# rpng/online_lang_splatting

Measured on AMD Instinct MI355X. Metric: rasterizer fwd+bwd frames/sec @500k Gaussians, 1200x680, 15-dim lang, higher is better.
Workload: dtype f32

## Files before the change

online_lang_splatting_amd/csrc/k_binning.hip:

```cpp
#include "olsr_device.h"
#include "olsr_kernels.h"
#include "olsr_loss_device.h"

namespace olsr {

constexpr int SCAN_THREADS = 256;
constexpr int SCAN_ITEMS = SCAN_CHUNK / SCAN_THREADS;

struct LoadPlain {
  const u32* p;
  __device__ __forceinline__ u32 operator()(int64_t i) const { return p[i]; }
};
struct LoadGather {
  const u32* vals;
  const u32* order;
  __device__ __forceinline__ u32 operator()(int64_t i) const { return vals[order[i]]; }
};

template <class Load>
__global__ __launch_bounds__(SCAN_THREADS) void scan_reduce_kernel(Load ld, int64_t n, u32* partials) {
  const int64_t base = (int64_t)blockIdx.x * SCAN_CHUNK + (int64_t)threadIdx.x * SCAN_ITEMS;
  u32 s = 0;
#pragma unroll
  for (int k = 0; k < SCAN_ITEMS; ++k)
// ... 324 lines not shown
    off[k] = run;
    run += n[k];
    nbig += (n[k] > EMIT_BIG) ? 1u : 0u;
    nmid += (n[k] > OLSR_MID_FOOTPRINT && n[k] <= EMIT_BIG) ? 1u : 0u;
  }
#pragma unroll
  for (int k = 0; k < EO_PER; ++k) {
    if (n[k] > 0) {
      inst_start[g[k]] = off[k];
      c_off[ci] = off[k];
      c_gid[ci] = g[k];
      for (u32 j = (off[k] + eb_out - 1u) >> eb_shift; (j << eb_shift) < off[k] + n[k]; ++j)
        win_start[j] = ci;
      ++ci;
    }
  }
  if ((r0 <= P - 1 && P - 1 < r0 + EO_PER) || (P == 0 && b == 0 && threadIdx.x == 0)) counters[CNT_EMITTERS] = (int32_t)ci;
  u32 slot = block_list_base<EO_T / 64>(nbig, &counters[CNT_BIG_LIST], s_lsum, &s_lbase);
#pragma unroll
  for (int k = 0; k < EO_PER; ++k)
    if (n[k] > EMIT_BIG) big_list[slot++] = make_uint4(g[k], off[k], n[k], 0u);
  u32 mslot = block_list_base<EO_T / 64>(nmid, &counters[CNT_MID_LIST], s_lsum, &s_lbase);
#pragma unroll
  for (int k = 0; k < EO_PER; ++k)
    if (n[k] > OLSR_MID_FOOTPRINT && n[k] <= EMIT_BIG) big_list[(u32)P_true - 1u - (mslot++)] = make_uint4(g[k], off[k], n[k], 0u);
}

struct EbGauss {
  float4 e0;
  float4 e1;
  uint4 m;
};

template <int TILE>
__global__ __launch_bounds__(EB_T) void emit_balanced_kernel(
    const u32* __restrict__ order, const u32* __restrict__ rank_off, const u32* __restrict__ win_start,
    const float4* __restrict__ emit_rec, int ellipse, int W, int H, int gx, const int32_t* __restrict__ counters,
    u32* __restrict__ keys, u32* __restrict__ inst_gid, u32 eb_out) {
  __shared__ EbGauss s_gs[EB_T];
  __shared__ u32 s_g[EB_T], s_first[EB_T], s_rowoff[EB_T];
  __shared__ uint8_t s_owner[EB_ROWCAP];
  __shared__ u32 s_w[EB_T / 64];
  __shared__ u32 s_flag;
  if (counters[CNT_OVERFLOW] != 0 || counters[CNT_SYNC_ERROR] != 0) return;
  const u32 R = (u32)counters[CNT_INSTANCES_EFF];
  const int P = counters[CNT_EMITTERS];
  const u32 o0 = blockIdx.x * eb_out;
  if (o0 >= R) return;
  const u32 o1 = min(o0 + eb_out, R);
  const int tid = threadIdx.x, lane = tid & 63;

  const int r_lo = (int)win_start[blockIdx.x];
  auto load_rank = [&](int r, u32& off, u32& end, u32& g) {
    off = 0; end = 0; g = 0;
    if (r < P) {
      off = rank_off[r];
      end = (r + 1 < P) ? rank_off[r + 1] : R;
      g = order[r];
    }
  };
  u32 off, end, g;
  load_rank(r_lo + tid, off, end, g);

  for (int rb0 = r_lo;; rb0 += EB_T) {
    const int r = rb0 + tid;
    const bool use = end > off && off < o1 && end > o0;
    u32 nrows = 0;
    if (use) {
      const float4 r0 = emit_rec[2 * (size_t)g], r1 = emit_rec[2 * (size_t)g + 1];
      const u32 yw = __float_as_uint(r1.z), xw = __float_as_uint(r1.w);
      nrows = yw >> 16;
      EbGauss q;
      q.m = make_uint4(0u, xw, yw & 0xFFFFu, off);
      q.e0 = make_float4(0.f, 0.f, 0.f, 0.f);
      q.e1 = make_float4(0.f, 0.f, 0.f, 0.f);
      if (ellipse) {
        const CullEllipse e = cull_setup(r0.x, r0.y, r0.z, r0.w, r1.x, r1.y, 0);
        q.e0 = make_float4(e.px, e.py, e.b, e.inv_a);
        q.e1 = make_float4(e.A, e.det_lo, e.xstar, e.ystar);
        q.m.x = e.exact ? 1u : 0u;
      }
      s_gs[tid] = q;
    }
// ... 25 lines not shown
          owner = (int)s_owner[idx - sbase];
          const EbGauss q = s_gs[owner];
          const int y = (int)q.m.z + (int)(idx - s_rowoff[owner]);
          int xa = (int)(q.m.y & 0xFFFFu), xb = (int)(q.m.y >> 16);
          if (ellipse) {
            CullEllipse e;
            e.px = q.e0.x; e.py = q.e0.y; e.b = q.e0.z; e.inv_a = q.e0.w;
            e.A = q.e1.x; e.det_lo = q.e1.y; e.xstar = q.e1.z; e.ystar = q.e1.w;
            e.ymax = 0.f;
            e.exact = q.m.x != 0u;
            cull_row_span<TILE>(e, xa, xb, y, W, H, xa, xb);
          }
          cnt = (u32)(xb - xa);
          key0 = (u32)(y * gx + xa);
        }
        u32 chunk_total;
        __syncthreads();
        const u32 S = carry + block_excl_scan<EB_T / 64>(cnt, s_w, &chunk_total);
        carry += chunk_total;
        if (live && idx == s_rowoff[owner]) s_first[owner] = S;
        __syncthreads();
        u32 out = 0, gid = 0;
        if (live) {
          out = s_gs[owner].m.w + (S - s_first[owner]);
          gid = s_g[owner];
        }
        const u32 jlo = max(out, o0), jhi = min(out + cnt, o1);
        const bool inside = live && jlo < jhi;
        if (inside && cnt <= EB_SHORT_ROW) {
          for (u32 j = jlo; j < jhi; ++j) {
            keys[j] = key0 + (j - out);
            inst_gid[j] = gid;
          }
        }
        u64 longrows = ballot(inside && cnt > EB_SHORT_ROW);
        while (longrows) {
          const int src = (int)__builtin_ctzll(longrows);
          longrows &= longrows - 1;
          const u32 lo_s = (u32)__shfl((int)jlo, src), hi_s = (u32)__shfl((int)jhi, src);
          const u32 out_s = (u32)__shfl((int)out, src), key_s = (u32)__shfl((int)key0, src);
          const u32 gid_s = (u32)__shfl((int)gid, src);
          for (u32 j = lo_s + (u32)lane; j < hi_s; j += 64) {
            keys[j] = key_s + (j - out_s);
            inst_gid[j] = gid_s;
          }
        }
      }
      __syncthreads();
    }
    if (!more) break;
    off = off_n;
    end = end_n;
    g = g_n;
    __syncthreads();
  }
}

__global__ __launch_bounds__(EMIT_THREADS) void emit_totals_kernel(int P, const u32* __restrict__ order,
                                                                   const u32* __restrict__ inst_count,
                                                                   u64* __restrict__ totals) {
  __shared__ u64 s_w[EMIT_THREADS / 64];
  const int r = (int)(blockIdx.x * EMIT_THREADS + threadIdx.x);
  u64 n = (r < P) ? emit_total_pack(inst_count[order[r]]) : 0ull;
  n = wave_sum(n);
  if ((threadIdx.x & 63) == 0) s_w[threadIdx.x >> 6] = n;
  __syncthreads();
  if (threadIdx.x == 0) {
    u64 t = 0;
    for (int i = 0; i < EMIT_THREADS / 64; ++i) t += s_w[i];
    totals[blockIdx.x] = t;
  }
}
void launch_emit_totals(const uint32_t* order, int P, const uint32_t* inst_count, uint32_t* emit_totals, hipStream_t st) {
  if (P <= 0) return;
  emit_totals_kernel<<<(P + EMIT_THREADS - 1) / EMIT_THREADS, EMIT_THREADS, 0, st>>>(P, order, inst_count,
                                                                                     reinterpret_cast<u64*>(emit_totals));
}

template <int TILE>
static void launch_emit_t(const olsr_scene& s, const FrameDims& d, const GeometryState& g, const BinningState& b,
                          int64_t bin_sync_words, int64_t n_host, const u32* order, const u32* alt_totals,
                          const u32* alt_unless, const int32_t* n_order_dev, hipStream_t st) {
  const int nb = (s.P + EMIT_THREADS - 1) / EMIT_THREADS;
  const int ellipse = (s.binning == OLSR_BINNING_ELLIPSE);
  const u32* totals = g.emit_status;
  uint4* bsync = reinterpret_cast<uint4*>(b.sync_words);
  const int quads = (int)((bin_sync_words + 3) / 4);
  u32* rank_off = g.key_b;
  u32* rank_gid = g.val_b;
  u32* win_start = b.key_b;
  const bool cut_mode = ellipse && s.tile_depth_cut != nullptr;
  const int eb_out = cut_mode ? EB_OUT / 4 : EB_OUT;
  emit_offsets_kernel<<<nb, EO_T, 0, st>>>(s.P, order, g.tiles_touched, g.counters, reinterpret_cast<const u64*>(totals), bsync,
                                           quads, rank_off, rank_gid, win_start, g.inst_start, g.big_list,
                                           (u32)__builtin_ctz((unsigned)eb_out), reinterpret_cast<const u64*>(alt_totals),
                                           alt_unless, n_order_dev);
  const int64_t nblk = (n_host + eb_out - 1) / eb_out;
  if (nblk > 0)
    emit_balanced_kernel<TILE><<<(int)nblk, EB_T, 0, st>>>(rank_gid, rank_off, win_start, g.emit_rec,
                                                           ellipse, d.W, d.H, d.gx, g.counters, b.key_a, b.inst_gid,
                                                           (u32)eb_out);
}

void launch_emit(const olsr_scene& s, const FrameDims& d, const GeometryState& g, const BinningState& b,
                 int64_t bin_sync_words, int64_t n_host, const uint32_t* order, const uint32_t* alt_totals,
                 const uint32_t* alt_unless, const int32_t* n_order_dev, hipStream_t st) {
  if (s.P <= 0) return;
  if (d.tile == 15) launch_emit_t<15>(s, d, g, b, bin_sync_words, n_host, order, alt_totals, alt_unless, n_order_dev, st);
  else launch_emit_t<16>(s, d, g, b, bin_sync_words, n_host, order, alt_totals, alt_unless, n_order_dev, st);
}

__device__ __forceinline__ void load_popc16(const uint8_t* __restrict__ flags, int64_t base, int64_t n, int shift,
                                            u32 mask, u32 (&v)[16]) {
  uint4 q = make_uint4(0u, 0u, 0u, 0u);
  if (base + 16 <= n) {
    q = *reinterpret_cast<const uint4*>(flags + base);
  } else {
    u32 w[4] = {0u, 0u, 0u, 0u};
    for (int k = 0; k < 16; ++k)
      if (base + k < n) w[k >> 2] |= (u32)flags[base + k] << (8 * (k & 3));
    q = make_uint4(w[0], w[1], w[2], w[3]);
  }
  const u32 w4[4] = {q.x, q.y, q.z, q.w};
#pragma unroll
  for (int k = 0; k < 16; ++k) v[k] = (u32)__popc((w4[k >> 2] >> (8 * (k & 3) + shift)) & mask);
}

constexpr int ROWS_THREADS = OLSR_ROWS_THREADS;
static_assert(ROWS_CHUNK == ROWS_THREADS * 16, "one 16-byte load of flags per thread");

struct RowCompactionArgs {
  const uint8_t* flags;
  int64_t n_host;
  const int32_t* n_dev;
  int shift;
  u32 mask;
  u32* rowbase;
  u32* status;
  u32* sync;
  long long row_capacity;
  int32_t* counters;
  int32_t* status_dev;
// ... 332 lines not shown
```

online_lang_splatting_amd/csrc/k_sort.hip:

```cpp
#include <cstdio>
#include <cstdlib>

#include "olsr_device.h"
#include "olsr_kernels.h"

namespace olsr {

constexpr u32 FS_READY = 0x80000000u;
constexpr int FS_T = FUSED_SORT_THREADS;
constexpr int FS_W = FS_T / 64;

typedef unsigned short u16;
constexpr u32 FS_READY16 = 0x8000u;
constexpr u32 FS_READY_PAIR = 0x80008000u;
typedef unsigned int u32x4 __attribute__((ext_vector_type(4)));
__device__ __forceinline__ bool fs_granule_ready(const u32x4& v) {
  return ((v.x & v.y & v.z & v.w) & FS_READY_PAIR) == FS_READY_PAIR;
}

struct FrameHousekeeping {
  const u32* part_rect;
  const u32* part_count;
  int nparts;
  long long capacity;
// ... 229 lines not shown

typedef __attribute__((address_space(3))) u32 lds_u32;
template <int DB>
__device__ __forceinline__ void wave_match_rank(u32 dg, bool valid, u32& rank, u32& pop) {
  const u64 vm = ballot(valid);
  u32 lo = (u32)vm, hi = (u32)(vm >> 32);
#pragma unroll
  for (int bit = 0; bit < DB; ++bit) {
    const u32 b = (dg >> bit) & 1u;
    const u64 bm = ballot(b != 0u);
    const u32 m = 0u - b;
    lo &= ~((u32)bm ^ m);
    hi &= ~((u32)(bm >> 32) ^ m);
  }
  rank = __builtin_amdgcn_mbcnt_hi(hi, __builtin_amdgcn_mbcnt_lo(lo, 0u));
  pop = (u32)__builtin_popcount(lo) + (u32)__builtin_popcount(hi);
}
__device__ __forceinline__ u32 lds_load(const u32* p) {
  return *reinterpret_cast<const volatile lds_u32*>((const lds_u32*)p);
}
__device__ __forceinline__ void lds_store(u32* p, u32 v) { *reinterpret_cast<volatile lds_u32*>((lds_u32*)p) = v; }

constexpr int FSF_IDENTITY = 1, FSF_NO_KEYS = 2, FSF_RANGES = 4, FSF_EMIT_TOTALS = 8;

template <int DB, int KPT, int T>
__global__ __launch_bounds__(T, (T == 1024 ? (KPT <= 2 ? 8 : 4) : (KPT <= 8 ? 8 : 6))) __attribute__((amdgpu_num_sgpr(80))) void sort_pass_kernel(const u32* __restrict__ keys_in,
                                                         const u32* __restrict__ vals_in, int64_t n_host,
                                                         const int32_t* __restrict__ n_dev, int shift,
                                                         const u32* __restrict__ ghist, u16* status, u32* ticket,
                                                         u32* __restrict__ keys_out, u32* __restrict__ vals_out,
                                                         int fsf, uint8_t* __restrict__ flags_clear, u32* ranges,
                                                         const u32* __restrict__ inst_count, u64* emit_totals,
                                                         unsigned long long* timing, int32_t* sync_error, int spin_limit,
                                                         int fault, const u32* __restrict__ run_if) {
  if (run_if != nullptr && __hip_atomic_load(run_if, __ATOMIC_RELAXED, __HIP_MEMORY_SCOPE_AGENT) == 0u) return;
  constexpr int TW = T / 64;
  static_assert(T == 1024 || T == 256, "block sizes of the radix passes");
  constexpr u32 NB = 1u << DB;
  static_assert((int)NB <= T, "a thread per digit");
  constexpr u32 DMASK = NB - 1u;
  constexpr int CHUNK = T * KPT;
  constexpr int C = (int)NB / 8;
  constexpr int RPB = T / C;
  constexpr int U = (DB <= 6) ? 4 : 8;
  extern __shared__ __attribute__((aligned(16))) u32 fs_smem[];
  u32* cnt = fs_smem;
  u32* dstart = cnt + TW * NB;
  u32* gbase = dstart + NB + 4;
  u16* pub = reinterpret_cast<u16*>(gbase + NB);
  u32* ex_key = gbase + NB + NB / 2;
  u32* ex_val = ex_key + CHUNK;
  __shared__ u32 s_bid;
  __shared__ u32 s_w[2 * TW];
  const int tid = threadIdx.x, lane = tid & 63, w = tid >> 6;
  if (tid == 0) s_bid = atomicAdd(ticket, 1u);
  for (u32 i = tid; i < TW * NB; i += T) cnt[i] = 0;
  const u32 gh = ((u32)tid < NB) ? ghist[tid] : 0u;
  const u32 gdig = block_excl_scan<TW>(gh, s_w);
  __syncthreads();
  const u32 b = s_bid;
  FS_STAMP(0);
  if (timing != nullptr && tid == 0) {
    timing[(size_t)b * 8 + 6] = (unsigned long long)(__builtin_amdgcn_s_getreg(63508) & 15);
    timing[(size_t)b * 8 + 7] = (unsigned long long)blockIdx.x;
  }
  const int64_t n = bounded_n(n_host, n_dev);
  const int64_t bbase = (int64_t)b * CHUNK;
  if (__hip_atomic_load(sync_error, __ATOMIC_RELAXED, __HIP_MEMORY_SCOPE_AGENT) != 0) return;
  if (b >= gridDim.x) {
    if (tid == 0) atomicOr(sync_error, 1);
    return;
  }
  if (bbase >= n) return;
  const int64_t wbase = bbase + (int64_t)w * (64 * KPT);

  u32 key[KPT], val[KPT];
#pragma unroll
  for (int r = 0; r < KPT; ++r) {
    const int64_t i = wbase + r * 64 + lane;
    const bool valid = i < n;
    key[r] = valid ? keys_in[i] : 0xFFFFFFFFu;
    val[r] = (fsf & FSF_IDENTITY) ? (u32)i : (valid ? vals_in[i] : 0u);
    if (valid) atomicAdd(&cnt[w * NB + ((key[r] >> shift) & DMASK)], 1u);
    if ((fsf & FSF_IDENTITY) && valid && flags_clear != nullptr) flags_clear[i] = 0;
  }
  __syncthreads();
  FS_STAMP(1);

  const u32 d = (u32)tid;
  u32 c[TW];
// ... 254 lines not shown
}

template <int KPT>
static void launch_sort_small_t(const u32* keys, int n, u32* vals_out, const u32* inst_count, u64* emit_totals,
                                const FrameHousekeeping& h, const u32* run_if, hipStream_t st) {
  constexpr size_t smem = sizeof(u32) * ((size_t)FS_W * 256 + 2 * (size_t)FS_T * KPT);
  static bool attr_set = false;
  if (!attr_set && smem > 64 * 1024) {
    (void)hipFuncSetAttribute(reinterpret_cast<const void*>(&sort_small_kernel<KPT>),
                              hipFuncAttributeMaxDynamicSharedMemorySize, (int)smem);
    attr_set = true;
  }
  sort_small_kernel<KPT><<<1, FS_T, smem, st>>>(keys, n, vals_out, inst_count, emit_totals, h, run_if);
}

struct PassArgs {
  const u32 *kin, *vin;
  int64_t n_host;
  const int32_t* n_dev;
  int shift;
  const u32* ghist;
  u16* status;
  u32* ticket;
  u32 *kout, *vout;
  int fsf;
  uint8_t* flags;
  u32* ranges;
  const u32* inst_count;
  u64* emit_totals;
  int nblk;
  int32_t* sync_error;
  int fault;
  const u32* run_if;
};

template <int DB, int KPT, int T>
static void launch_pass_t(const PassArgs& a, hipStream_t st) {
  constexpr size_t NB = 1u << DB;
  constexpr size_t smem = sizeof(u32) * ((T / 64) * NB + NB + 4 + NB + NB / 2 + 2 * (size_t)T * KPT);
  static bool attr_set = false;
  if (!attr_set && smem > 64 * 1024) {
    (void)hipFuncSetAttribute(reinterpret_cast<const void*>(&sort_pass_kernel<DB, KPT, T>),
                              hipFuncAttributeMaxDynamicSharedMemorySize, (int)smem);
    attr_set = true;
  }
  static bool printed = std::getenv("OLSR_SORT_DEBUG") == nullptr;
  if (!printed) {
    int nb = -1;
    (void)hipOccupancyMaxActiveBlocksPerMultiprocessor(&nb, sort_pass_kernel<DB, KPT, T>, T, smem);
    std::fprintf(stderr, "[olsr] sort_pass_kernel<%d,%d,%d>: %zu B dynamic LDS, occupancy API: %d blocks/CU, grid %d\n", DB,
                 KPT, T, smem, nb, a.nblk);
    printed = true;
  }
  unsigned long long* timing = nullptr;
  if (g_timing.buf && g_timing.launch < g_timing.max_launches && a.nblk <= g_timing.max_blocks)
    timing = g_timing.buf + (size_t)(g_timing.launch++) * g_timing.max_blocks * 8;
  sort_pass_kernel<DB, KPT, T><<<a.nblk, T, smem, st>>>(a.kin, a.vin, a.n_host, a.n_dev, a.shift, a.ghist, a.status,
                                                        a.ticket, a.kout, a.vout, a.fsf, a.flags, a.ranges,
                                                        a.inst_count, a.emit_totals, timing, a.sync_error,
                                                        sort_knobs().spin_limit.load(std::memory_order_relaxed), a.fault,
                                                        a.run_if);
}

template <int DB, int T>
static void launch_pass_kt(int kpt, const PassArgs& a, hipStream_t st) {
  switch (kpt) {
    case 2: launch_pass_t<DB, 2, T>(a, st); break;
    case 4: launch_pass_t<DB, 4, T>(a, st); break;
    case 8: launch_pass_t<DB, 8, T>(a, st); break;
    case 12: launch_pass_t<DB, 12, T>(a, st); break;
    default: launch_pass_t<DB, 16, T>(a, st); break;
  }
}
template <int DB>
static void launch_pass_k(const SortPlan& plan, const PassArgs& a, hipStream_t st) {
  if (plan.threads == 256) launch_pass_kt<DB, 256>(plan.kpt, a, st);
  else launch_pass_kt<DB, 1024>(plan.kpt, a, st);
}

int fused_sort_digit_bits(int bits, int* passes_out) {
  const int passes = (bits + 7) / 8;
  int db = (bits + passes - 1) / passes;
  if (db < 4) db = 4;
  if (passes_out) *passes_out = passes;
  return db;
}

bool fused_sort_applicable(int64_t n_host, int bits) {
  return n_host > 0 && bits <= 32 && fused_sort_fits(n_host);
}

static FrameHousekeeping housekeeping_of(const FusedHouse* house) {
  FrameHousekeeping h{};
  if (house) {
// ... 35 lines not shown
}

void launch_sort_hist(const uint32_t* keys, int64_t n_host, const int32_t* n_dev, int bits, uint32_t* hist,
                      const FusedHouse* house, int threads, hipStream_t st, const uint32_t* run_if,
                      const SortCompaction* compaction) {
  int passes;
  const int db = fused_sort_digit_bits(bits, &passes);
  const FrameHousekeeping h = housekeeping_of(house);
  const int T = threads;
  int64_t nb = (n_host + (int64_t)T * 4 - 1) / ((int64_t)T * 4);
  if (nb < 1) nb = 1;
#ifndef OLSR_HIST_BLOCKS
#define OLSR_HIST_BLOCKS 256
#endif
  if (nb > OLSR_HIST_BLOCKS) nb = OLSR_HIST_BLOCKS;
  CompactArgs ca{};
  size_t smem = 0;
  if (compaction != nullptr) {
    ca.inst_count = compaction->inst_count;
    ca.part_vis = compaction->part_vis;
    ca.nparts = (int)((n_host + 255) / 256);
    ca.out_keys = compaction->out_keys;
    ca.out_gid = compaction->out_gid;
    ca.n_out = compaction->n_out;
    smem = sizeof(u32) * (size_t)ca.nparts;
  }
  if (T == 256) sort_hist_kernel<256><<<(int)nb, 256, smem, st>>>(keys, n_host, n_dev, passes, db, hist, h, house ? 1 : 0, run_if, ca);
  else sort_hist_kernel<1024><<<(int)nb, 1024, smem, st>>>(keys, n_host, n_dev, passes, db, hist, h, house ? 1 : 0, run_if, ca);
}

int launch_sort_fused(const SortBuffers& b, const SortPlan& plan, int64_t n_host, const int32_t* n_dev, int bits,
                      bool vals_in_identity, const uint32_t* hist, uint32_t* status, uint32_t* tickets, uint8_t* flags_clear, uint32_t* ranges,
                      const uint32_t* inst_count, uint32_t* emit_totals, int32_t* sync_error, int fault, hipStream_t st,
                      uint32_t* final_vals_out, const uint32_t* run_if) {
  if (n_host <= 0) return 0;
  int passes;
  const int db = fused_sort_digit_bits(bits, &passes);
  const size_t NB = (size_t)1 << db;
  u32 *kin = b.key_a, *kout = b.key_b, *vin = b.val_a, *vout = b.val_b;
  int where = 0;
  for (int p = 0; p < passes; ++p) {
    int fsf = 0;
    if (p == 0 && vals_in_identity) fsf |= FSF_IDENTITY;
    if (p == passes - 1) fsf |= FSF_NO_KEYS | (ranges ? FSF_RANGES : 0) | (emit_totals ? FSF_EMIT_TOTALS : 0);
    PassArgs a{kin, vin, n_host, n_dev, db * p, hist + 256 * p,
               reinterpret_cast<u16*>(status) + (size_t)p * plan.nblk * NB, tickets + p, kout,
               (p == passes - 1 && final_vals_out != nullptr) ? final_vals_out : vout, fsf, flags_clear,
               ranges, inst_count, reinterpret_cast<u64*>(emit_totals), plan.nblk, sync_error, p == 0 ? fault : 0, run_if};
    switch (db) {
      case 4: launch_pass_k<4>(plan, a, st); break;
      case 5: launch_pass_k<5>(plan, a, st); break;
      case 6: launch_pass_k<6>(plan, a, st); break;
      case 7: launch_pass_k<7>(plan, a, st); break;
      case 8: launch_pass_k<8>(plan, a, st); break;
      default: break;
    }
    u32* t = kin; kin = kout; kout = t;
    t = vin; vin = vout; vout = t;
    where ^= 1;
  }
  return where;
}

}
```

online_lang_splatting_amd/csrc/olsr_api.hip:

```cpp
#include <hip/hip_runtime.h>

#include <algorithm>
#include <string>

#include "olsr_device.h"
#include "olsr_host.h"

using namespace olsr;

namespace {
thread_local std::string g_err;
}

int olsr::fail(int code, const std::string& msg) {
  g_err = msg;
  return code;
}

namespace {

int check_scene(const olsr_scene* s, bool backward) {
  if (!s) return fail(OLSR_ERR_ARG, "scene is NULL");
  if (s->P < 0) return fail(OLSR_ERR_ARG, "P must be >= 0");
  if (s->width <= 0 || s->height <= 0) return fail(OLSR_ERR_ARG, "image size must be positive");
// ... 129 lines not shown
      launch_emit_totals(g.depth_order, s.P, g.tiles_touched, g.emit_status, st);
    }
    STAGE(s, "depth_sort", st);
    }
  }

  void* bin_buf = nullptr;
  if (!sync_mode) {
    n_host = c.capacity;
    bin_buf = c.bin_buf;
  } else {
    int32_t R = 0;
    if (s.P > 0) OLSR_TRY(pinned_count_wait(st, &R));
    n_host = R;
    if (c.num_rendered_host) *c.num_rendered_host = R;
    bin_buf = c.bin_alloc(c.bin_user, olsr_binning_bytes(R, s.F));
    if (!bin_buf) return fail(OLSR_ERR_ALLOC, "binning allocation callback returned NULL");
  }
  const BinningState b = BinningState::carve(bin_buf, (size_t)n_host);
  const int32_t* n_dev = &g.counters[CNT_INSTANCES_EFF];

  if (s.P > 0) {
    const int tbits = tile_bits(d.ntiles);
    int tpasses = 0;
    const int tdb = fused_sort_digit_bits(tbits, &tpasses);
    const bool fused_tiles = !legacy && fused_sort_applicable(n_host, tbits);
    const bool cut_mode = !sync_mode && s.tile_depth_cut != nullptr && s.binning == OLSR_BINNING_ELLIPSE;
    const SortPlan tile_plan = sort_plan(n_host, !sync_mode, cut_mode ? 25 : 85,
                                         (s.flags & OLSR_FLAG_FRAMES_IN_FLIGHT) != 0);
    const int64_t bin_sync_words =
        (b.tile_status - b.sync_words) +
        (fused_tiles ? ((int64_t)tpasses * tile_plan.nblk * ((int64_t)1 << tdb) + 1) / 2 : 0);
    launch_emit(s, d, g, b, bin_sync_words, n_host, carry ? carry : (order ? order : g.depth_order),
                carry ? g.carry_totals : nullptr, carry ? g.carry_miss : nullptr, n_order_dev, st);
    STAGE(s, "emit", st);
    if (n_host > 0) {
      const bool odd = tile_sort_where(d.ntiles) != 0;
      SortBuffers sb{b.key_a, b.key_b, odd ? b.val_b : b.src, odd ? b.src : b.val_b, b.radix_table, b.scan_partials};
      if (fused_tiles) {
        launch_sort_hist(b.key_a, n_host, n_dev, tbits, b.tile_hist, nullptr, tile_plan.threads, st);
        launch_sort_fused(sb, tile_plan, n_host, n_dev, tbits, true, b.tile_hist, b.tile_status, b.tickets + BT_TILE_PASS, b.flags,
                          im.ranges, nullptr, nullptr, &g.counters[CNT_SYNC_ERROR],
                          sort_knobs().fault.load(std::memory_order_relaxed) & 2, st);
      } else {
        const int where = launch_radix_sort(sb, n_host, n_dev, tbits, true, st);
        launch_tile_ranges(where ? b.key_b : b.key_a, n_host, n_dev, im.ranges, b.flags, st);
      }
      STAGE(s, "tile_sort", st);
    }
  }
  ForwardTail tail;
  uint32_t* tile_order_inout = c.tile_order_inout;
  if (sync_mode) OLSR_TRY(rows_ring_post(st, tail));
  if (c.view_hints != nullptr && s.P > 0) {
    tail.hint_slot = c.view_hints;
    tile_order_inout = c.view_hints + HINT_HDR;
  }
  if (s.backward_row_capacity > 0 && s.P > 0 && bin_buf != nullptr) tail.compact_rows_n = n_host;
  stamp(st, 0);
  launch_render_forward(s, d, g, b, im, c.out_color, c.out_language, c.out_depth, c.out_opacity, c.n_touched, tile_order_inout,
                        c.num_rendered_dev, (s.P > 0) ? c.loss : nullptr, tail, st);
  stamp(st, 1);
  STAGE(s, "render_forward", st);

  if (c.num_rendered_dev && s.P == 0) HIP_TRY(hipMemsetAsync(c.num_rendered_dev, 0, 2 * sizeof(int32_t), st));
  return OLSR_OK;
}

}

extern "C" {

const char* olsr_last_error(void) { return g_err.c_str(); }

const char* olsr_version(void) { return "olsr 0.1 (gfx950)"; }

// ... 246 lines not shown
```

online_lang_splatting_amd/csrc/olsr_diag.hip:

```cpp
#include <hip/hip_runtime.h>

#include <cstdlib>
#include <cstring>
#include <vector>

#include "olsr_device.h"
#include "olsr_host.h"

using namespace olsr;

namespace {

thread_local bool g_profiling = false;
struct StageMark {
  const char* name;
  hipEvent_t ev;
};
thread_local std::vector<StageMark> g_marks;

void marks_reset() {
  for (auto& m : g_marks) (void)hipEventDestroy(m.ev);
  g_marks.clear();
}

// ... 81 lines not shown

const void* olsr_geometry_field(const void* geometry_buffer, int32_t P, int32_t F, const char* name) {
  const GeometryState g = GeometryState::carve(const_cast<void*>(geometry_buffer), (size_t)P, grad_row(supported_F(F) ? F : 0));
  if (!std::strcmp(name, "depths")) return g.depths;
  if (!std::strcmp(name, "means2D")) return g.means2D;
  if (!std::strcmp(name, "cov3D")) return g.cov3D;
  if (!std::strcmp(name, "conic_opacity")) return g.conic_opacity;
  if (!std::strcmp(name, "rgb")) return g.rgb;
  if (!std::strcmp(name, "clamped")) return g.clamped;
  if (!std::strcmp(name, "tiles_touched")) return g.tiles_touched;
  if (!std::strcmp(name, "depth_order")) return g.depth_order;
  if (!std::strcmp(name, "depth_order_compacted")) return g.gacc;
  if (!std::strcmp(name, "counters")) return g.counters;
  if (!std::strcmp(name, "emit_totals")) return g.emit_status;
  if (!std::strcmp(name, "inst_start")) return g.inst_start;
  if (!std::strcmp(name, "blended")) return g.blended;
  if (!std::strcmp(name, "carry_miss")) return g.carry_miss;
  if (!std::strcmp(name, "carry_totals")) return g.carry_totals;
  if (!std::strcmp(name, "sort_keys")) return g.key_a;
  return nullptr;
}

const void* olsr_binning_field(const void* binning_buffer, int64_t num_rendered, int32_t F, const char* name) {
  (void)F;
  const BinningState b = BinningState::carve(const_cast<void*>(binning_buffer), (size_t)num_rendered);
  if (!std::strcmp(name, "inst_gid")) return b.inst_gid;
  if (!std::strcmp(name, "flags")) return b.flags;
  if (!std::strcmp(name, "rowbase")) return b.rowbase;
  if (!std::strcmp(name, "row_sync")) return b.tickets + BT_ROWS;
  if (!std::strcmp(name, "key_a")) return b.key_a;
  if (!std::strcmp(name, "key_b")) return b.key_b;
  if (!std::strcmp(name, "src")) return b.src;
  if (!std::strcmp(name, "val_b")) return b.val_b;
  return nullptr;
}

const void* olsr_image_field(const void* image_buffer, int32_t width, int32_t height, int32_t tile, const char* name) {
  const ImageState im =
      ImageState::carve(const_cast<void*>(image_buffer), (size_t)width * height, tile_count(width, height, tile));
  if (!std::strcmp(name, "final_T")) return im.final_T;
  if (!std::strcmp(name, "n_contrib")) return im.n_contrib;
  if (!std::strcmp(name, "ranges")) return im.ranges;
  if (!std::strcmp(name, "tile_work")) return im.tile_work;
  if (!std::strcmp(name, "tile_order")) return im.tile_order;
  return nullptr;
}

void olsr_set_profiling(int enable) {
  g_profiling = enable != 0;
  marks_reset();
}

int olsr_get_stage_times(const char** names, float* ms, int max) {
  if (g_marks.size() < 2) return 0;
  (void)hipEventSynchronize(g_marks.back().ev);
  int n = 0;
  for (size_t i = 1; i < g_marks.size() && n < max; ++i) {
    if (!std::strcmp(g_marks[i].name, "begin")) continue;
    float t = 0.f;
    if (hipEventElapsedTime(&t, g_marks[i - 1].ev, g_marks[i].ev) != hipSuccess) t = -1.f;
    names[n] = g_marks[i].name;
    ms[n] = t;
    ++n;
  }
  return n;
}
// ... 67 lines not shown
```

online_lang_splatting_amd/csrc/olsr_kernels.h:

```cpp
#pragma once
#include <hip/hip_runtime.h>
#include <stdint.h>

#include "../../include/olsr.h"
#include "olsr_state.h"

namespace olsr {

constexpr uint32_t OLSR_BIG_FOOTPRINT = 32;
constexpr uint32_t OLSR_MID_FOOTPRINT = 12;

struct FrameDims {
  int W, H, tile, gx, gy, ntiles;
  float focal_x, focal_y;
};

void launch_preprocess(const olsr_scene& s, const FrameDims& d, const GeometryState& g, int32_t* radii,
                       int32_t* n_touched, hipStream_t st);
void launch_mark_visible(int P, const float* means3D, const float* view, uint8_t* present, hipStream_t st);

struct SortBuffers {
  uint32_t *key_a, *key_b, *val_a, *val_b, *table, *partials;
};
int launch_radix_sort(const SortBuffers& b, int64_t n_host, const int32_t* n_dev, int bits, bool vals_in_identity,
                      hipStream_t st);
void launch_emit(const olsr_scene& s, const FrameDims& d, const GeometryState& g, const BinningState& b,
                 int64_t bin_sync_words, int64_t n_host, const uint32_t* order, const uint32_t* alt_totals,
                 const uint32_t* alt_unless, const int32_t* n_order_dev, hipStream_t st);
void launch_row_compaction(const uint8_t* flags, int64_t n_host, const int32_t* n_dev, bool packed_ref15,
                           uint32_t* rowbase, uint32_t* row_status, uint32_t* sync, int64_t row_capacity,
                           int32_t* counters, int32_t* status_dev, hipStream_t st);
struct LossFinalArgs {
  const float* partials;
  int nb, W, H, F, has_lang;
  float alpha, lamda;
  float* loss;
  float* d_exposure;
  int use_exposure, zero_exposure;
};
struct ForwardTailRows {
  const uint8_t* flags;
  int64_t n_host;
  const int32_t* n_dev;
  bool packed_ref15;
  uint32_t* rowbase;
  uint32_t* row_status;
  uint32_t* sync;
  int64_t row_capacity;
  int32_t* counters;
};
void launch_tile_order(const uint32_t* tile_work, uint32_t* tile_order, uint32_t* order_copy, int ntiles,
                       uint32_t* live_rows, int32_t* rows_mailbox, int32_t rows_seq, const int32_t* counters,
                       int32_t* num_rendered_dev, int32_t* sticky_error, const uint32_t* hint_slot, float* depth_cut,
                       int gx, int gy, const LossFinalArgs& loss_final, const ForwardTailRows* rows, hipStream_t st);
void launch_tile_ranges(const uint32_t* sorted_keys, int64_t n_host, const int32_t* n_dev, uint32_t* ranges,
                        uint8_t* flags, hipStream_t st);

struct FusedHouse {
  const uint32_t* part_rect;
  const uint32_t* part_count;
  int nparts;
  long long capacity;
  int32_t* counters;
  int32_t* num_rendered_dev;
  uint32_t* ranges;
  int nranges;
  int32_t* host_mailbox;
  int32_t host_seq;
  uint32_t* live_rows;
  uint32_t* hint_base;
  const float* view;
};
constexpr int HINT_SLOTS = 16;
constexpr int HINT_HDR = 4 + HINT_SLOTS + 16 * HINT_SLOTS;
static_assert(HINT_HDR % 4 == 0, "the orders stay 16-byte aligned");
constexpr float HINT_VIEW_TOL = 0.03f;
bool fused_sort_applicable(int64_t n_host, int bits);
int fused_sort_digit_bits(int bits, int* passes_out);
struct SortCompaction {
  const uint32_t* inst_count;
  const uint32_t* part_vis;
  uint32_t* out_keys;
  uint32_t* out_gid;
  int32_t* n_out;
};
bool depth_sort_compaction_applicable(int64_t P);
void launch_sort_hist(const uint32_t* keys, int64_t n_host, const int32_t* n_dev, int bits, uint32_t* hist,
                      const FusedHouse* house, int threads , hipStream_t st,
                      const uint32_t* run_if = nullptr, const SortCompaction* compaction = nullptr);
int launch_sort_fused(const SortBuffers& b, const SortPlan& plan, int64_t n_host, const int32_t* n_dev, int bits,
                      bool vals_in_identity, const uint32_t* hist, uint32_t* status, uint32_t* tickets, uint8_t* flags_clear, uint32_t* ranges,
                      const uint32_t* inst_count, uint32_t* emit_totals, int32_t* sync_error, int fault, hipStream_t st,
                      uint32_t* final_vals_out = nullptr, const uint32_t* run_if = nullptr);
void debug_set_sort_timing(unsigned long long* buf, int max_blocks, int max_launches);
bool small_depth_sort_applicable(int64_t n, bool as_fallback = false);
void launch_small_depth_sort(const uint32_t* keys, int n, uint32_t* order_out, const uint32_t* inst_count,
                             uint32_t* emit_totals, const FusedHouse* house, const uint32_t* run_if, hipStream_t st);
void launch_order_repair(int P, uint32_t* carry, const uint32_t* keys, uint32_t* tmp_key, uint32_t* tmp_gid,
                         const uint32_t* inst_count, uint32_t* totals, uint32_t* miss, bool frames_in_flight,
                         hipStream_t st);
void launch_emit_totals(const uint32_t* order, int P, const uint32_t* inst_count, uint32_t* emit_totals, hipStream_t st);

struct ForwardTail {
  int32_t* rows_dev = nullptr;
  int32_t rows_seq = 0;
  int32_t* sticky = nullptr;
  const uint32_t* hint_slot = nullptr;
  int64_t compact_rows_n = -1;
};

void launch_render_forward(const olsr_scene& s, const FrameDims& d, const GeometryState& g, const BinningState& b,
                           const ImageState& im, float* out_color, float* out_language, float* out_depth,
                           float* out_opacity, int32_t* n_touched, uint32_t* tile_order_inout, int32_t* num_rendered_dev,
                           const olsr_loss_fusion* loss, const ForwardTail& tail, hipStream_t st);

void launch_render_backward_reference(const olsr_scene& s, int F_rows, const FrameDims& d, const GeometryState& g,
                                      const BinningState& b, const ImageState& im, const float* dL_dcolor,
                                      const float* dL_dlanguage, const float* dL_ddepth, float* rows, hipStream_t st);
void launch_render_backward_exact(const olsr_scene& s, int F_rows, const FrameDims& d, const GeometryState& g,
                                  const BinningState& b, const ImageState& im, const float* dL_dcolor,
                                  const float* dL_dlanguage, const float* dL_ddepth, float* rows, hipStream_t st);

void launch_render_backward_ordered(const olsr_scene& s, const FrameDims& d, const GeometryState& g, const BinningState& b,
                                    const ImageState& im, int64_t num_rendered, const float* dL_dcolor,
                                    const float* dL_dlanguage, const float* dL_ddepth, float* rows, uint8_t* used,
                                    float* dL_dmean2D, float* dL_dconic, float* dL_dopacity, float* dL_dcolors,
// ... 110 lines not shown
```

online_lang_splatting_amd/csrc/olsr_state.h:

```cpp
#pragma once
#include <hip/hip_runtime.h>
#include <stddef.h>
#include <stdint.h>
#include <atomic>
#include <cstdlib>

namespace olsr {

constexpr size_t ALIGN = 256;
inline size_t align_up(size_t v) { return (v + ALIGN - 1) / ALIGN * ALIGN; }
template <typename T = void>
inline T* align_ptr(const void* p) { return reinterpret_cast<T*>(align_up(reinterpret_cast<uintptr_t>(p))); }

constexpr int SORT_CHUNK = 4096;
constexpr int SCAN_CHUNK = 4096;
inline int sort_blocks(long long n) { return (int)((n + SORT_CHUNK - 1) / SORT_CHUNK); }
inline int scan_blocks(long long n) { return (int)((n + SCAN_CHUNK - 1) / SCAN_CHUNK); }

struct SortPlan {
  int kpt;
  int nblk;
  int threads;
};
constexpr int FUSED_SORT_THREADS = 1024;
// ... 25 lines not shown
  const long long res = sort_plan_resident_blocks() * (1024 / T);
  const long long n_est = n_is_capacity ? (n * fill_pct + 99) / 100 : n;
  int best = sort_plan_forced_kpt();
  if (best == 2 && T == 256) best = 4;
  if (best != 0 && (n + T * best - 1) / (T * best) > FUSED_SORT_MAX_BLOCKS) best = 0;
  if (best == 0 && T == 256) best = 16;
  if (best == 0) {
    double best_cost = 0.0;
    for (int i = (T == 256 ? 1 : 0); i < 5; ++i) {
      const long long chunk = T * cand[i];
      if ((n + chunk - 1) / chunk > FUSED_SORT_MAX_BLOCKS && i < 4) continue;
      const long long nb = (n_est + chunk - 1) / chunk;
      const double cost = (double)((nb + res - 1) / res) * (cand[i] + 11.0) + (T == 256 ? (double)nb / 128.0 : 0.0);
      if (best == 0 || cost < best_cost) {
        best = cand[i];
        best_cost = cost;
      }
    }
  }
  return SortPlan{best, (int)((n + T * best - 1) / (T * best)), (int)T};
}
inline bool fused_sort_fits(long long n) { return (n + 4095) / 4096 <= FUSED_SORT_MAX_BLOCKS; }
inline size_t fused_status_words(long long n, int passes) {
  if (!fused_sort_fits(n)) return 0;
  long long nb = (n + 1023) / 1024;
  if (nb > FUSED_SORT_MAX_BLOCKS) nb = FUSED_SORT_MAX_BLOCKS;
  return (size_t)passes * (size_t)nb * 128;
}
constexpr int EMIT_CHUNK = 1024;
constexpr int EMIT_TOTAL_SHIFT = 40;
__host__ __device__ inline unsigned long long emit_total_pack(uint32_t instances) {
  return (unsigned long long)instances | ((unsigned long long)(instances != 0u) << EMIT_TOTAL_SHIFT);
}
#ifndef OLSR_ROWS_THREADS
#define OLSR_ROWS_THREADS 1024
#endif
constexpr int ROWS_CHUNK = 16 * OLSR_ROWS_THREADS;

struct Carver {
  char* base;
  size_t off = 0;
  explicit Carver(void* b) : base(b ? align_ptr<char>(b) : nullptr) {}
  template <typename T>
  T* take(size_t count) {
    off = align_up(off);
    T* p = base ? (T*)(base + off) : nullptr;
    off += count * sizeof(T);
    return p;
  }
  size_t total() const { return align_up(off) + ALIGN; }
};

enum Counter {
  CNT_INSTANCES = 0,
  CNT_INSTANCES_EFF = 1,
  CNT_OVERFLOW = 2,
  CNT_RECT_INSTANCES = 3,
  CNT_MID_LIST = 4,
  CNT_BIG_LIST = 5,
  CNT_LIVE_ROWS = 6,
  CNT_ROW_OVERFLOW = 7,
  CNT_SYNC_ERROR = 8,
  CNT_CUT_MISS = 9,
  CNT_EMITTERS = 10,
  CNT_ROWS_STAMP = 11,
  CNT_SORTED = 12,
// ... 112 lines not shown

struct BinningState {
  uint32_t* key_a;
  uint32_t* key_b;
  uint32_t* val_b;
  uint32_t* src;
  uint32_t* inst_gid;
  uint8_t* flags;
  uint32_t* radix_table;
  uint32_t* scan_partials;
  uint32_t* rowbase;
  uint32_t* sync_words;
  size_t sync_count;
  uint32_t* tickets;
  uint32_t* tile_hist;
  uint32_t* tile_status;
  uint32_t* row_status;
  static BinningState carve(void* buf, size_t R, size_t* bytes = nullptr) {
    Carver c(buf);
    BinningState b;
    b.key_a = c.take<uint32_t>(R);
    b.key_b = c.take<uint32_t>(R);
    b.val_b = c.take<uint32_t>(R);
    b.src = c.take<uint32_t>(R);
    b.inst_gid = c.take<uint32_t>(R);
    b.flags = c.take<uint8_t>((R + 15) / 16 * 16);
    const size_t table = 256 * (size_t)sort_blocks((long long)R);
    b.radix_table = c.take<uint32_t>(table);
    b.scan_partials = c.take<uint32_t>((size_t)scan_blocks((long long)(table > R ? table : R)) + 1);
    b.rowbase = c.take<uint32_t>(R + 1);
    {
      const size_t st_words = fused_status_words((long long)R, 4);
      const size_t row_blocks = 2 * ((R + 1 + ROWS_CHUNK - 1) / ROWS_CHUNK + 1);
      b.sync_count = TICKET_WORDS + 4 * 256 + st_words + row_blocks;
      b.sync_count = (b.sync_count + 3) / 4 * 4;
      b.sync_words = c.take<uint32_t>(b.sync_count);
      b.tickets = b.sync_words;
      b.tile_hist = b.tickets + TICKET_WORDS;
      b.row_status = b.tile_hist + 4 * 256;
      b.tile_status = b.row_status + row_blocks;
    }
    if (bytes) *bytes = c.total();
    return b;
  }
};

}
```

Baseline: 2495.

## Fuse tile-key radix histogram into emit kernel, drop separate histogram pass

```diff
diff --git a/online_lang_splatting_amd/csrc/k_binning.hip b/online_lang_splatting_amd/csrc/k_binning.hip
--- a/online_lang_splatting_amd/csrc/k_binning.hip
+++ b/online_lang_splatting_amd/csrc/k_binning.hip
@@ -380,11 +380,35 @@
   uint4 m;
 };
 
+__device__ __forceinline__ void count_key_run(u32* s_hist, u32 a, u32 b, u32 lane, u32 lanes, int db, int passes) {
+  const u32 NB = 1u << db, mask = NB - 1u;
+  if (lane == 0u) {
+    const u32 L = b - a, s0 = a & mask, r = L & mask;
+    if (L >> db) atomicAdd(&s_hist[(u32)passes << db], L >> db);
+    if (r != 0u) {
+      atomicAdd(&s_hist[s0], 1u);
+      const u32 e = s0 + r;
+      if (e > NB) atomicAdd(&s_hist[0], 1u);
+      if (e != NB) atomicAdd(&s_hist[e & mask], 0xFFFFFFFFu);
+    }
+  }
+  for (int p = 1; p < passes; ++p) {
+    const int sh = db * p;
+    const u32 q0 = a >> sh, nseg = ((b - 1u) >> sh) - q0 + 1u;
+    for (u32 i = lane; i < nseg; i += lanes) {
+      const u32 q = q0 + i;
+      const u32 lo = max(a, q << sh), hi = min(b, (q + 1u) << sh);
+      atomicAdd(&s_hist[((u32)p << db) + (q & mask)], hi - lo);
+    }
+  }
+}
 template <int TILE>
 __global__ __launch_bounds__(EB_T) void emit_balanced_kernel(
     const u32* __restrict__ order, const u32* __restrict__ rank_off, const u32* __restrict__ win_start,
     const float4* __restrict__ emit_rec, int ellipse, int W, int H, int gx, const int32_t* __restrict__ counters,
-    u32* __restrict__ keys, u32* __restrict__ inst_gid, u32 eb_out) {
+    u32* __restrict__ keys, u32* __restrict__ inst_gid, u32 eb_out, u32* __restrict__ tile_hist, int hist_db,
+    int hist_passes) {
+  extern __shared__ u32 s_hist[];
   __shared__ EbGauss s_gs[EB_T];
   __shared__ u32 s_g[EB_T], s_first[EB_T], s_rowoff[EB_T];
   __shared__ uint8_t s_owner[EB_ROWCAP];
@@ -397,6 +421,9 @@
   if (o0 >= R) return;
   const u32 o1 = min(o0 + eb_out, R);
   const int tid = threadIdx.x, lane = tid & 63;
+  const bool counting = tile_hist != nullptr;
+  if (counting)
+    for (int i = tid; i <= (hist_passes << hist_db); i += EB_T) s_hist[i] = 0u;
 
   const int r_lo = (int)win_start[blockIdx.x];
   auto load_rank = [&](int r, u32& off, u32& end, u32& g) {
@@ -488,6 +515,7 @@
             keys[j] = key0 + (j - out);
             inst_gid[j] = gid;
           }
+          if (counting) count_key_run(s_hist, key0 + (jlo - out), key0 + (jhi - out), 0u, 1u, hist_db, hist_passes);
         }
         u64 longrows = ballot(inside && cnt > EB_SHORT_ROW);
         while (longrows) {
@@ -500,6 +528,7 @@
             keys[j] = key_s + (j - out_s);
             inst_gid[j] = gid_s;
           }
+          if (counting) count_key_run(s_hist, key_s + (lo_s - out_s), key_s + (hi_s - out_s), (u32)lane, 64u, hist_db, hist_passes);
         }
       }
       __syncthreads();
@@ -509,6 +538,21 @@
     end = end_n;
     g = g_n;
     __syncthreads();
+  }
+  if (counting) {
+    __syncthreads();
+    const u32 diff = tid < (1 << hist_db) ? s_hist[tid] : 0u;
+    const u32 met = block_excl_scan<EB_T / 64>(diff, s_w) + diff + s_hist[hist_passes << hist_db];
+    __syncthreads();
+    if (tid < (1 << hist_db)) s_hist[tid] = met;
+    __syncthreads();
+    u32* copy = tile_hist + (size_t)(blockIdx.x & (u32)(TILE_HIST_COPIES - 1)) * TILE_HIST_WORDS;
+    for (int i = tid; i < (hist_passes << hist_db); i += EB_T) {
+      const u32 c = s_hist[i];
+      if (c != 0u)
+        __hip_atomic_fetch_add(&copy[(i >> hist_db) * 256 + (i & ((1 << hist_db) - 1))], c, __ATOMIC_RELAXED,
+                               __HIP_MEMORY_SCOPE_AGENT);
+    }
   }
 }
 
@@ -536,8 +580,11 @@
 template <int TILE>
 static void launch_emit_t(const olsr_scene& s, const FrameDims& d, const GeometryState& g, const BinningState& b,
                           int64_t bin_sync_words, int64_t n_host, const u32* order, const u32* alt_totals,
-                          const u32* alt_unless, const int32_t* n_order_dev, hipStream_t st) {
+                          const u32* alt_unless, const int32_t* n_order_dev, u32* tile_hist, int hist_db, int hist_passes,
+                          hipStream_t st) {
   const int nb = (s.P + EMIT_THREADS - 1) / EMIT_THREADS;
+  if (hist_passes > 4 || hist_db > 8) tile_hist = nullptr;
+  const size_t hist_lds = tile_hist != nullptr ? sizeof(u32) * (((size_t)hist_passes << hist_db) + 1) : 0;
   const int ellipse = (s.binning == OLSR_BINNING_ELLIPSE);
   const u32* totals = g.emit_status;
   uint4* bsync = reinterpret_cast<uint4*>(b.sync_words);
@@ -553,17 +600,20 @@
                                            alt_unless, n_order_dev);
   const int64_t nblk = (n_host + eb_out - 1) / eb_out;
   if (nblk > 0)
-    emit_balanced_kernel<TILE><<<(int)nblk, EB_T, 0, st>>>(rank_gid, rank_off, win_start, g.emit_rec,
-                                                           ellipse, d.W, d.H, d.gx, g.counters, b.key_a, b.inst_gid,
-                                                           (u32)eb_out);
+    emit_balanced_kernel<TILE><<<(int)nblk, EB_T, hist_lds, st>>>(rank_gid, rank_off, win_start, g.emit_rec,
+                                                                  ellipse, d.W, d.H, d.gx, g.counters, b.key_a, b.inst_gid,
+                                                                  (u32)eb_out, tile_hist, hist_db, hist_passes);
 }
 
 void launch_emit(const olsr_scene& s, const FrameDims& d, const GeometryState& g, const BinningState& b,
                  int64_t bin_sync_words, int64_t n_host, const uint32_t* order, const uint32_t* alt_totals,
-                 const uint32_t* alt_unless, const int32_t* n_order_dev, hipStream_t st) {
+                 const uint32_t* alt_unless, const int32_t* n_order_dev, uint32_t* tile_hist, int hist_db, int hist_passes,
+                 hipStream_t st) {
   if (s.P <= 0) return;
-  if (d.tile == 15) launch_emit_t<15>(s, d, g, b, bin_sync_words, n_host, order, alt_totals, alt_unless, n_order_dev, st);
-  else launch_emit_t<16>(s, d, g, b, bin_sync_words, n_host, order, alt_totals, alt_unless, n_order_dev, st);
+  if (d.tile == 15)
+    launch_emit_t<15>(s, d, g, b, bin_sync_words, n_host, order, alt_totals, alt_unless, n_order_dev, tile_hist, hist_db, hist_passes, st);
+  else
+    launch_emit_t<16>(s, d, g, b, bin_sync_words, n_host, order, alt_totals, alt_unless, n_order_dev, tile_hist, hist_db, hist_passes, st);
 }
 
 __device__ __forceinline__ void load_popc16(const uint8_t* __restrict__ flags, int64_t base, int64_t n, int shift,
diff --git a/online_lang_splatting_amd/csrc/k_sort.hip b/online_lang_splatting_amd/csrc/k_sort.hip
--- a/online_lang_splatting_amd/csrc/k_sort.hip
+++ b/online_lang_splatting_amd/csrc/k_sort.hip
@@ -285,7 +285,7 @@
                                                          int fsf, uint8_t* __restrict__ flags_clear, u32* ranges,
                                                          const u32* __restrict__ inst_count, u64* emit_totals,
                                                          unsigned long long* timing, int32_t* sync_error, int spin_limit,
-                                                         int fault, const u32* __restrict__ run_if) {
+                                                         int fault, const u32* __restrict__ run_if, int hist_copies) {
   if (run_if != nullptr && __hip_atomic_load(run_if, __ATOMIC_RELAXED, __HIP_MEMORY_SCOPE_AGENT) == 0u) return;
   constexpr int TW = T / 64;
   static_assert(T == 1024 || T == 256, "block sizes of the radix passes");
@@ -308,7 +308,16 @@
   const int tid = threadIdx.x, lane = tid & 63, w = tid >> 6;
   if (tid == 0) s_bid = atomicAdd(ticket, 1u);
   for (u32 i = tid; i < TW * NB; i += T) cnt[i] = 0;
-  const u32 gh = ((u32)tid < NB) ? ghist[tid] : 0u;
+  u32 gh = 0u;
+  if ((u32)tid < NB) {
+    for (int c0 = 0; c0 < hist_copies; c0 += 8) {
+      u32 part[8];
+#pragma unroll
+      for (int k = 0; k < 8; ++k) part[k] = (c0 + k < hist_copies) ? ghist[(size_t)(c0 + k) * TILE_HIST_WORDS + tid] : 0u;
+#pragma unroll
+      for (int k = 0; k < 8; ++k) gh += part[k];
+    }
+  }
   const u32 gdig = block_excl_scan<TW>(gh, s_w);
   __syncthreads();
   const u32 b = s_bid;
@@ -629,6 +638,7 @@
   int32_t* sync_error;
   int fault;
   const u32* run_if;
+  int hist_copies;
 };
 
 template <int DB, int KPT, int T>
@@ -656,7 +666,7 @@
                                                         a.ticket, a.kout, a.vout, a.fsf, a.flags, a.ranges,
                                                         a.inst_count, a.emit_totals, timing, a.sync_error,
                                                         sort_knobs().spin_limit.load(std::memory_order_relaxed), a.fault,
-                                                        a.run_if);
+                                                        a.run_if, a.hist_copies);
 }
 
 template <int DB, int T>
@@ -758,7 +768,7 @@
 int launch_sort_fused(const SortBuffers& b, const SortPlan& plan, int64_t n_host, const int32_t* n_dev, int bits,
                       bool vals_in_identity, const uint32_t* hist, uint32_t* status, uint32_t* tickets, uint8_t* flags_clear, uint32_t* ranges,
                       const uint32_t* inst_count, uint32_t* emit_totals, int32_t* sync_error, int fault, hipStream_t st,
-                      uint32_t* final_vals_out, const uint32_t* run_if) {
+                      uint32_t* final_vals_out, const uint32_t* run_if, int hist_copies) {
   if (n_host <= 0) return 0;
   int passes;
   const int db = fused_sort_digit_bits(bits, &passes);
@@ -772,7 +782,8 @@
     PassArgs a{kin, vin, n_host, n_dev, db * p, hist + 256 * p,
                reinterpret_cast<u16*>(status) + (size_t)p * plan.nblk * NB, tickets + p, kout,
                (p == passes - 1 && final_vals_out != nullptr) ? final_vals_out : vout, fsf, flags_clear,
-               ranges, inst_count, reinterpret_cast<u64*>(emit_totals), plan.nblk, sync_error, p == 0 ? fault : 0, run_if};
+               ranges, inst_count, reinterpret_cast<u64*>(emit_totals), plan.nblk, sync_error, p == 0 ? fault : 0, run_if,
+               hist_copies};
     switch (db) {
       case 4: launch_pass_k<4>(plan, a, st); break;
       case 5: launch_pass_k<5>(plan, a, st); break;
diff --git a/online_lang_splatting_amd/csrc/olsr_api.hip b/online_lang_splatting_amd/csrc/olsr_api.hip
--- a/online_lang_splatting_amd/csrc/olsr_api.hip
+++ b/online_lang_splatting_amd/csrc/olsr_api.hip
@@ -185,16 +185,16 @@
         (b.tile_status - b.sync_words) +
         (fused_tiles ? ((int64_t)tpasses * tile_plan.nblk * ((int64_t)1 << tdb) + 1) / 2 : 0);
     launch_emit(s, d, g, b, bin_sync_words, n_host, carry ? carry : (order ? order : g.depth_order),
-                carry ? g.carry_totals : nullptr, carry ? g.carry_miss : nullptr, n_order_dev, st);
+                carry ? g.carry_totals : nullptr, carry ? g.carry_miss : nullptr, n_order_dev, fused_tiles ? b.tile_hist : nullptr,
+                tdb, tpasses, st);
     STAGE(s, "emit", st);
     if (n_host > 0) {
       const bool odd = tile_sort_where(d.ntiles) != 0;
       SortBuffers sb{b.key_a, b.key_b, odd ? b.val_b : b.src, odd ? b.src : b.val_b, b.radix_table, b.scan_partials};
       if (fused_tiles) {
-        launch_sort_hist(b.key_a, n_host, n_dev, tbits, b.tile_hist, nullptr, tile_plan.threads, st);
         launch_sort_fused(sb, tile_plan, n_host, n_dev, tbits, true, b.tile_hist, b.tile_status, b.tickets + BT_TILE_PASS, b.flags,
                           im.ranges, nullptr, nullptr, &g.counters[CNT_SYNC_ERROR],
-                          sort_knobs().fault.load(std::memory_order_relaxed) & 2, st);
+                          sort_knobs().fault.load(std::memory_order_relaxed) & 2, st, nullptr, nullptr, TILE_HIST_COPIES);
       } else {
         const int where = launch_radix_sort(sb, n_host, n_dev, tbits, true, st);
         launch_tile_ranges(where ? b.key_b : b.key_a, n_host, n_dev, im.ranges, b.flags, st);
diff --git a/online_lang_splatting_amd/csrc/olsr_diag.hip b/online_lang_splatting_amd/csrc/olsr_diag.hip
--- a/online_lang_splatting_amd/csrc/olsr_diag.hip
+++ b/online_lang_splatting_amd/csrc/olsr_diag.hip
@@ -137,6 +137,8 @@
   if (!std::strcmp(name, "key_b")) return b.key_b;
   if (!std::strcmp(name, "src")) return b.src;
   if (!std::strcmp(name, "val_b")) return b.val_b;
+  if (!std::strcmp(name, "tile_hist")) return b.tile_hist;
+  if (!std::strcmp(name, "row_status")) return b.row_status;
   return nullptr;
 }
 
diff --git a/online_lang_splatting_amd/csrc/olsr_kernels.h b/online_lang_splatting_amd/csrc/olsr_kernels.h
--- a/online_lang_splatting_amd/csrc/olsr_kernels.h
+++ b/online_lang_splatting_amd/csrc/olsr_kernels.h
@@ -26,7 +26,8 @@
                       hipStream_t st);
 void launch_emit(const olsr_scene& s, const FrameDims& d, const GeometryState& g, const BinningState& b,
                  int64_t bin_sync_words, int64_t n_host, const uint32_t* order, const uint32_t* alt_totals,
-                 const uint32_t* alt_unless, const int32_t* n_order_dev, hipStream_t st);
+                 const uint32_t* alt_unless, const int32_t* n_order_dev, uint32_t* tile_hist, int hist_db, int hist_passes,
+                 hipStream_t st);
 void launch_row_compaction(const uint8_t* flags, int64_t n_host, const int32_t* n_dev, bool packed_ref15,
                            uint32_t* rowbase, uint32_t* row_status, uint32_t* sync, int64_t row_capacity,
                            int32_t* counters, int32_t* status_dev, hipStream_t st);
@@ -91,7 +92,7 @@
 int launch_sort_fused(const SortBuffers& b, const SortPlan& plan, int64_t n_host, const int32_t* n_dev, int bits,
                       bool vals_in_identity, const uint32_t* hist, uint32_t* status, uint32_t* tickets, uint8_t* flags_clear, uint32_t* ranges,
                       const uint32_t* inst_count, uint32_t* emit_totals, int32_t* sync_error, int fault, hipStream_t st,
-                      uint32_t* final_vals_out = nullptr, const uint32_t* run_if = nullptr);
+                      uint32_t* final_vals_out = nullptr, const uint32_t* run_if = nullptr, int hist_copies = 1);
 void debug_set_sort_timing(unsigned long long* buf, int max_blocks, int max_launches);
 bool small_depth_sort_applicable(int64_t n, bool as_fallback = false);
 void launch_small_depth_sort(const uint32_t* keys, int n, uint32_t* order_out, const uint32_t* inst_count,
diff --git a/online_lang_splatting_amd/csrc/olsr_state.h b/online_lang_splatting_amd/csrc/olsr_state.h
--- a/online_lang_splatting_amd/csrc/olsr_state.h
+++ b/online_lang_splatting_amd/csrc/olsr_state.h
@@ -81,6 +81,12 @@
 __host__ __device__ inline unsigned long long emit_total_pack(uint32_t instances) {
   return (unsigned long long)instances | ((unsigned long long)(instances != 0u) << EMIT_TOTAL_SHIFT);
 }
+#ifndef OLSR_TILE_HIST_COPIES
+#define OLSR_TILE_HIST_COPIES 8
+#endif
+constexpr int TILE_HIST_COPIES = OLSR_TILE_HIST_COPIES;
+constexpr int TILE_HIST_WORDS = 4 * 256;
+static_assert(TILE_HIST_COPIES >= 1 && (TILE_HIST_COPIES & (TILE_HIST_COPIES - 1)) == 0, "a power of two");
 #ifndef OLSR_ROWS_THREADS
 #define OLSR_ROWS_THREADS 1024
 #endif
@@ -259,12 +265,12 @@
     {
       const size_t st_words = fused_status_words((long long)R, 4);
       const size_t row_blocks = 2 * ((R + 1 + ROWS_CHUNK - 1) / ROWS_CHUNK + 1);
-      b.sync_count = TICKET_WORDS + 4 * 256 + st_words + row_blocks;
+      b.sync_count = TICKET_WORDS + (size_t)TILE_HIST_COPIES * TILE_HIST_WORDS + st_words + row_blocks;
       b.sync_count = (b.sync_count + 3) / 4 * 4;
       b.sync_words = c.take<uint32_t>(b.sync_count);
       b.tickets = b.sync_words;
       b.tile_hist = b.tickets + TICKET_WORDS;
-      b.row_status = b.tile_hist + 4 * 256;
+      b.row_status = b.tile_hist + (size_t)TILE_HIST_COPIES * TILE_HIST_WORDS;
       b.tile_status = b.row_status + row_blocks;
     }
     if (bytes) *bytes = c.total();
```

After: 2498 (median of 3 runs). No clear change (+0.1%).
